# jiaxi98/cnf_ot

Hardware: AMD Instinct MI355X
Metric: MC samples/sec through flow fwd+log|detJ| at dim=2, batch=65536 (higher is better)
Workload: dtype f32; 1 GPU; configs[1]: OT free dim=2, batch=65536, sample_and_log_prob (RQS fwd + log|detJ|), L=2 H=16 M=2 K=5, params N(0,0.20^2) seed 42; ONE STEP = one evaluator-shaped pass of 10000 time-slices x 65536 samples (cnf_ot/utils.py:311-340), each slice its own condition t, one cnf_sample_logprob call per rank; batch=65536, dim=2, parallelism=slice-shard x1 (contiguous blocks of the step's slices; no collective)

## Files before the change

cnf_ot_amd/csrc/cnf_flow.hip:

```cpp
#include "cnf_flow_tile.h"
#include "cnf_host.h"
#include "cnf_pwl_build.h"

#include <math.h>
#include <new>
#include <stdlib.h>
#include <string.h>

namespace cnf {

__global__ void circular_slopes_kernel(const float* __restrict__ params, float* __restrict__ prep, int K, int H,
                                       int D, int L, int M, int64_t per_layer) {
  const int P = 3 * K + 1;
  const int hdr = hdr_floats(K);
  const int l = blockIdx.x / (D - 1), d = 1 + blockIdx.x % (D - 1);
  int64_t o = (int64_t)l * per_layer;
  for (int dd = 1; dd < d; ++dd) o += cond_floats_p(dd, H, M, P, true);
  o += cond_floats_p(d, H, M, P, true) - ((int64_t)H * P + P);
  for (int r = threadIdx.x; r <= H; r += blockDim.x)
    prep[hdr + o + (int64_t)r * P + 3 * K] = params[P + o + (int64_t)r * P + 2 * K];
}

__global__ void prepare_kernel(const float* __restrict__ params, float* __restrict__ prep,
                               int K, int64_t n_params, double lo, double hi, double min_bin,
// ... 213 lines not shown
      const bool odd = l & 1;
      const int first_idx = odd ? D - 1 : 0, idx_step = odd ? -1 : 1;
      const float* cu = U + SPL * lane;
      float* co = O + SPL * lane;
      T o, ld;
      if (wave == 0) {
        table_spline<K, true, FAST, T>(tab, lds_get<T>(cu, first_idx, TS), sc, o, ld);
        lds_put(co, first_idx, TS, o);
        acc += ld;
      }
      for (int d = 1 + wave; d < D; d += NW) {
        const int64_t off = l * a.m.per_layer + (int64_t)H * ((d - 1) + (int64_t)d * (d - 1) / 2) + (d - 1) * cpart;
        T th[P];
        conditioner<H, P, T>(weights + off, d, a.m.M, c, cu, first_idx, idx_step, TS, th);
        const int idx = first_idx + d * idx_step;
        cond_spline<K, true, FAST, T>(th, lds_get<T>(cu, idx, TS), sc, o, ld);
        lds_put(co, idx, TS, o);
        acc += ld;
      }
      __syncthreads();
      float* t = U; U = O; O = t;
    }
    if (a.aux) lds_put(LD + wave * TS + SPL * lane, 0, TS, acc);
    __syncthreads();
    if (a.aux && wave == 0) {
      T tot = splat<T>(0.0f);
      for (int w = 0; w < NW; ++w) tot += lds_get<T>(LD + w * TS + SPL * lane, 0, TS);
      store_aux(a.aux, i, a.B, a.aux_mode == AUX_LOGPROB ? base - tot : tot);
    }
    if (a.out) tile_store_n<float>(a.out, U, D, a.div_magic, TS, tile_start, a.B, NT);
  }
}

struct PwlArgs {
  ModelArgs m;
  const float* in;
  float* out;
  float* aux;
  const float* tables;
  int64_t B, slice_len;
  int32_t n_slices, tiles_per_slice, aux_mode;
  const uint32_t* gate;
  uint32_t gate_epoch;
  int32_t gate_want;
  uint64_t seed;
  int64_t first_sample, slice_stride;
  int32_t in_shared;
};

__global__ void cond_uniform_kernel(const float* __restrict__ c, int64_t B, uint32_t* flag, uint32_t epoch) {
  const uint32_t c0 = __float_as_uint(c[0]);
  bool diff = false;
  for (int64_t i = blockIdx.x * (int64_t)blockDim.x + threadIdx.x; i < B; i += (int64_t)gridDim.x * blockDim.x)
    diff |= __float_as_uint(c[i]) != c0;
  if (__syncthreads_or(diff) && threadIdx.x == 0) *flag = epoch;
}

template <int K, bool TO_BASE, bool FAST, bool PRECISE = false, int LROWS = PWL_LROWS, int LFIX = 0, bool SEEDED = false>
__global__ __launch_bounds__(PWL_MAX_THREADS) void flow_pwl_kernel(const PwlArgs a) {
  const int PWL_THREADS = blockDim.x, PWL_TS = 2 * PWL_THREADS;
  extern __shared__ __attribute__((aligned(16))) float lds_raw[];
  constexpr int HDR = (hdr_floats(K) + 3) & ~3;
  float* tab = lds_raw;
  float* tbl = lds_raw + HDR;
  const int tid = threadIdx.x;
  const int L = LFIX ? LFIX : a.m.L;
  if (gate_closed(a)) return;
  for (int i = tid; i < hdr_floats(K); i += PWL_THREADS) tab[i] = table_of<float>(a.m)[i];
  const SplineConsts sc = sc_scalars(sc_of<float>(a.m));
  [[maybe_unused]] double* e2tab = nullptr;
  [[maybe_unused]] double* tabd = nullptr;
  if constexpr (PRECISE) {
    e2tab = reinterpret_cast<double*>(tbl + L * pwl_ltbl(LROWS));
    tabd = e2tab + EXP2_N;
    for (int i = tid; i < EXP2_N; i += PWL_THREADS) e2tab[i] = a.m.e2tab[i];
    for (int i = tid; i < hdr_floats(K); i += PWL_THREADS) tabd[i] = a.m.tabd[i];
  }

  const int total = a.n_slices * a.tiles_per_slice;
  const int per_block = (total + gridDim.x - 1) / gridDim.x;
  const int t0 = blockIdx.x * per_block;
  const int t1 = t0 + per_block < total ? t0 + per_block : total;
  int cur = -1;
  struct Tile { int slice; int ti; int valid; int64_t g0; int64_t st0; int64_t gin; };
  auto tile_at = [&](int slice, int ti) {
    Tile t;
    t.slice = slice;
    t.ti = ti;
    const int64_t s0 = (int64_t)t.slice * a.slice_len;
    const int64_t len = a.B - s0 < a.slice_len ? a.B - s0 : a.slice_len;
    const int64_t jt = (int64_t)ti * PWL_TS;
    const int64_t left = len - jt;
    t.valid = left >= PWL_TS ? PWL_TS : (left > 0 ? (int)left : 0);
    t.g0 = s0 + jt;
    t.gin = a.in_shared ? jt : t.g0;
    t.st0 = a.first_sample + (int64_t)t.slice * a.slice_stride + jt;
    return t;
  };
  auto tile_of = [&](int tile) { const int sl = tile / a.tiles_per_slice; return tile_at(sl, tile - sl * a.tiles_per_slice); };
  auto tile_next = [&](const Tile& t) {
    return t.ti + 1 < a.tiles_per_slice ? tile_at(t.slice, t.ti + 1) : tile_at(t.slice + 1, 0);
  };
  const uint32_t lane2 = 2u * (uint32_t)tid;
  auto tile_points = [&](const Tile& t) {
    f4 x = {0.f, 0.f, 0.f, 0.f};
    if (SEEDED && !a.in) {
      const uint64_t e0 = (uint64_t)(t.st0 + lane2) * 2u;
      if ((int)lane2 < t.valid) {
        if ((e0 & 3) == 0) {
          float z[4];
          philox_normals4(a.seed, e0 >> 2, z);
#pragma unroll
          for (int q = 0; q < 4; ++q) x[q] = z[q];
        } else {
#pragma unroll
          for (int q = 0; q < 4; ++q) x[q] = normal_at(a.seed, e0 + q);
        }
        if ((int)lane2 + 1 >= t.valid) { x[2] = 0.f; x[3] = 0.f; }
      }
      return x;
    }
    const float* p = a.in + 2 * t.gin;
    if (t.valid == PWL_TS) x = *reinterpret_cast<const f4*>(p + 2u * lane2);
    else if ((int)lane2 + 1 < t.valid) x = *reinterpret_cast<const f4*>(p + 2u * lane2);
    else if ((int)lane2 < t.valid) { x[0] = p[2u * lane2]; x[1] = p[2u * lane2 + 1]; }
    return x;
  };
  [[maybe_unused]] f4 xn = {0.f, 0.f, 0.f, 0.f};
  Tile tn{};
  if (t0 < t1) { tn = tile_of(t0); xn = tile_points(tn); }
  for (int tile = t0; tile < t1; ++tile) {
    const Tile tl = tn;
    const int slice = tl.slice;
    if (slice != cur) {
      __syncthreads();
      pwl_stage<LROWS>(tbl, a.tables + (int64_t)slice * L * PWL_TBL, L, tid, PWL_THREADS);
      cur = slice;
      __syncthreads();
    }
    const bool full = tl.valid == PWL_TS;
    const bool v0 = (int)lane2 < tl.valid, v1 = (int)lane2 + 1 < tl.valid;
    const f4 x = xn;
    if (tile + 1 < t1) { tn = tile_next(tl); xn = tile_points(tn); }
    __builtin_amdgcn_sched_barrier(0);
    v2f u0 = {x[0], x[2]}, u1 = {x[1], x[3]};
    [[maybe_unused]] v2f poison = splat<v2f>(0.0f);
    if constexpr (TO_BASE) poison = (u0 - u0) + (u1 - u1);

    v2f base = splat<v2f>(0.0f);
    if (!TO_BASE && a.aux_mode == AUX_LOGPROB && a.aux) base = (u0 * u0 + u1 * u1) * -0.5f - (float)(2 * HALF_LOG_2PI);
    BaseAcc<v2f> bacc;
    const v2f acc = flow2_tables<K, TO_BASE, FAST, PRECISE, true, LROWS, LFIX, true>(tab, tbl, a.tables + (int64_t)slice * L * PWL_TBL, L, sc,
                                                            u0, u1, &a.m.scd, e2tab, tabd, &bacc);
    if (a.aux) {
      v2f r = acc;
      if constexpr (PRECISE) { if (a.aux_mode == AUX_LOGPROB) r = bacc.log_prob(acc, 2); }
      else if (a.aux_mode == AUX_LOGPROB)
        r = TO_BASE ? (u0 * u0 + u1 * u1) * -0.5f - (float)(2 * HALF_LOG_2PI) + acc : base - acc;
      if constexpr (TO_BASE) r += poison;
      float* q = a.aux + tl.g0;
      if (full || v1) *reinterpret_cast<v2f*>(q + lane2) = r;
      else if (v0) q[lane2] = r.x;
    }
    if (a.out) {
      float* q = a.out + 2 * tl.g0;
      if constexpr (TO_BASE) { u0 += poison; u1 += poison; }
      if (full || v1) *reinterpret_cast<f4*>(q + 2u * lane2) = f4{u0.x, u1.x, u0.y, u1.y};
      else if (v0) { q[2u * lane2] = u0.x; q[2u * lane2 + 1] = u1.x; }
    }
  }
}

struct LossArgs {
  ModelArgs m;
  CnfLossSpec spec;
  const float* pts;
  const float* t;
  double* sums;
  int64_t B;
  int64_t n_slices;
  int64_t pts_slice_stride;
  uint32_t div_magic;
  uint64_t seed;
  int64_t first_sample;
  DensityMix mix;
};

template <class T>
__device__ __forceinline__ void copy_cols(float* dst, const float* src, int D, int TS) {
  for (int d = 0; d < D; ++d) lds_put(dst, d, TS, lds_get<T>(src, d, TS));
}

__device__ __forceinline__ float mask_tail(float v, int64_t i, int64_t B) { return i < B ? v : 0.0f; }
__device__ __forceinline__ float mask_tail(v2f v, int64_t i, int64_t B) {
  return (i < B ? v.x : 0.0f) + (i + 1 < B ? v.y : 0.0f);
}

template <int H, int K, bool FAST, class T>
__global__ __launch_bounds__(TILE, 2) void loss_kernel(const LossArgs a) {
  extern __shared__ __attribute__((aligned(16))) float lds[];
  constexpr int HDR = hdr_floats(K);
  constexpr int SPL = Lanes<T>::N;
  constexpr int TS = TILE * SPL;
  using M = Math<FAST>;
  const int D = a.m.D;
  float* tab = lds;
  float* Nn = lds + HDR;
  float* U = Nn + D * TS;
  float* O = U + D * TS;
  float* V = O + D * TS;
  float* R = V + D * TS;
  for (int i = threadIdx.x; i < HDR; i += TILE) tab[i] = a.m.prep[i];
  const int col = SPL * threadIdx.x;
  const int kind = a.spec.kind;

  const int64_t tiles_per_slice = (a.B + TS - 1) / TS;
  const int64_t n_tiles = tiles_per_slice * a.n_slices;
  SliceSum ssum;
  for (int64_t tile = blockIdx.x; tile < n_tiles; tile += gridDim.x) {
    const int64_t slice = tile / tiles_per_slice;
    const int64_t tile_start = (tile - slice * tiles_per_slice) * TS;
    const int64_t i = tile_start + col;
    __syncthreads();
    if (a.pts)
      tile_load<float>(a.pts + slice * a.pts_slice_stride * D, Nn, D, a.div_magic, TS, tile_start, a.B);
    else
      tile_noise(a.seed, (uint64_t)(a.first_sample + slice * a.pts_slice_stride + tile_start) * (uint64_t)D, Nn, D,
                 a.div_magic, TS, a.B - tile_start);
    const float t = a.t[slice];
    __syncthreads();

    T acc = splat<T>(0.0f);
    const float dt = a.spec.dt;
    const bool kin = kind <= CNF_TERM_FLOW_MATCHING;
    const bool data = kind == CNF_TERM_NEG_LOGPROB || kind == CNF_TERM_DENSITY_L2_DATA;
    const int n_fwd = data ? 0 : (kind == CNF_TERM_KINETIC ? 2 : (kin ? 3 : 1));
    T fldj = splat<T>(0.0f);
    for (int p = 0; p < n_fwd; ++p) {
      const float c = !kin ? t : (p == 0 ? t - 0.5f * dt : (p == 1 ? t + 0.5f * dt : t));
      copy_cols<T>(U + col, Nn + col, D, TS);
      fldj = flow_pass<H, K, false, FAST, T>(a.m, tab, U, O, splat<T>(c));
      if (kin) {
        if (p == 0) copy_cols<T>(V + col, U + col, D, TS);
        else if (p == 1) {
          const float inv_dt = 1.0f / dt;
          for (int d = 0; d < D; ++d)
            lds_put(V + col, d, TS, (lds_get<T>(U + col, d, TS) - lds_get<T>(V + col, d, TS)) * inv_dt);
        } else copy_cols<T>(R + col, U + col, D, TS);
      }
    }
    if (kind == CNF_TERM_KINETIC) {
// ... 448 lines not shown
                  spl == 2 ? CNF_PATH_MLP2 : CNF_PATH_MLP1, gated, a.B);
  });
}

struct SlicePlan { int64_t tps, chunk; float* tables; };

static int slice_plan(CnfModel* m, hipStream_t stream, int64_t slice_len, int64_t n_slices, int64_t tile,
                      int sets_per_slice, SlicePlan* p) {
  const int64_t PWL_MAX_SLICES = 2048;
  p->tps = (slice_len + tile - 1) / tile;
  const int64_t total = n_slices * p->tps;
  if (total > (1 << 30)) return CNF_ERR_UNSUPPORTED;
  if (m->use_pwl == 1 && (total < 2 * (int64_t)m->num_cus || slice_len < 4 * tile)) return CNF_ERR_UNSUPPORTED;
  p->chunk = n_slices < PWL_MAX_SLICES ? n_slices : PWL_MAX_SLICES;
  int64_t sets = 0;
  pwl_workspace(m, stream, &p->tables, &sets);
  if (sets / sets_per_slice < p->chunk) p->chunk = sets / sets_per_slice;
  if (p->chunk < 1) return CNF_ERR_UNSUPPORTED;
  if (m->use_pwl == 1 && p->chunk < n_slices && p->chunk * p->tps < (int64_t)m->num_cus) return CNF_ERR_UNSUPPORTED;
  return CNF_OK;
}

constexpr int64_t PWL_LEAN_MIN_TABLES = 2048;
static void build_tables(CnfModel* m, hipStream_t stream, const float* c, float offset, int64_t ns, float* tables) {
  const int L = m->cfg.num_layers;
  const float* w = m->prep + cnf::hdr_floats(5);
  const bool lean = m->pwl_builder == 0 ? ns * L >= PWL_LEAN_MIN_TABLES : m->pwl_builder != 1;
  m->last_pwl_builder = lean ? 2 : 1;
  const dim3 grid((unsigned)(ns * L));
  if (!lean)
    hipLaunchKernelGGL(cnf::pwl_build_kernel, grid, dim3(512), 0, stream, w, m->per_layer, c, offset, L,
                       m->scd.sp_offset, tables);
  else
    hipLaunchKernelGGL(cnf::pwl_build_lean_kernel<64>, grid, dim3(64), 0, stream, w, m->per_layer, c, offset, L,
                       m->scd.sp_offset, tables);
}

typedef void (*PwlKernel)(const cnf::PwlArgs);

template <bool TO_BASE, bool PRECISE, bool SEEDED>
static PwlKernel flow_pwl_kernel_of(bool full, bool l2) {
  constexpr int ALL = cnf::PWL_NPIECE, WIN = cnf::PWL_LROWS;
  if (l2) return cnf::flow_pwl_kernel<5, TO_BASE, true, PRECISE, ALL, 2, SEEDED>;
  return full ? cnf::flow_pwl_kernel<5, TO_BASE, true, PRECISE, ALL, 0, SEEDED>
              : cnf::flow_pwl_kernel<5, TO_BASE, true, PRECISE, WIN, 0, SEEDED>;
}
static PwlKernel flow_pwl_kernel_of(bool to_base, bool precise, bool seeded, bool full, bool l2) {
  if (precise) return flow_pwl_kernel_of<true, true, false>(full, l2);
  if (to_base) return flow_pwl_kernel_of<true, false, false>(full, l2);
  return seeded ? flow_pwl_kernel_of<false, false, true>(full, l2) : flow_pwl_kernel_of<false, false, false>(full, l2);
}

struct NoiseSrc { uint64_t seed; int64_t first_sample, slice_stride; };

static int run_flow_pwl(CnfModel* m, bool to_base, const float* in, const float* c, int64_t c_block,
                        float* out, float* aux, int aux_mode, int64_t B, hipStream_t stream,
                        bool detect = false, const uint32_t** gate = nullptr, uint32_t* gate_epoch = nullptr,
                        const NoiseSrc* noise = nullptr, const float* built = nullptr, bool in_shared = false) {
  if (!pwl_config_ok(m)) return CNF_ERR_UNSUPPORTED;
  const int L = m->cfg.num_layers;
  const bool precise = to_base && m->precise;
  auto lds_for = [&](int lrows) {
    return (size_t)(((cnf::hdr_floats(5) + 3) & ~3) + L * cnf::pwl_ltbl(lrows)) * sizeof(float) +
           (precise ? precise_lds_bytes(5) : 0);
  };
  const bool full = lds_for(cnf::PWL_NPIECE) <= 160 * 1024;
  size_t lds = lds_for(full ? cnf::PWL_NPIECE : cnf::PWL_LROWS);
  if (lds > 160 * 1024) return CNF_ERR_UNSUPPORTED;
  const int64_t slice_len = c_block < B ? c_block : B;
  const int64_t n_slices = (B + slice_len - 1) / slice_len;
  if (n_slices > 1 && (slice_len & 1)) return CNF_ERR_UNSUPPORTED;
  if ((reinterpret_cast<uintptr_t>(in) & 15) || (reinterpret_cast<uintptr_t>(out) & 15) ||
      (reinterpret_cast<uintptr_t>(aux) & 7))
    return CNF_ERR_UNSUPPORTED;
  const int pwl_threads = cnf::PWL_MAX_THREADS;
  const size_t pwl_min_lds = 82 * 1024;
  SlicePlan plan;
  if (slice_plan(m, stream, slice_len, n_slices, 2 * pwl_threads, 1, &plan) != CNF_OK) return CNF_ERR_UNSUPPORTED;
  const int64_t tps = plan.tps, chunk = plan.chunk;
  float* tables = plan.tables;
  if (built && (chunk < n_slices || built != tables)) return CNF_ERR_UNSUPPORTED;
  if (pwl_min_lds > lds) lds = pwl_min_lds;
  const PwlKernel kern = flow_pwl_kernel_of(to_base, precise, noise != nullptr, full, full && L == 2);
  if (!ensure_lds(kern, lds)) return CNF_ERR_UNSUPPORTED;
  uint32_t* flag = nullptr;
  uint32_t epoch = 0;
  if (detect) {
    int64_t sets = 0;
    pwl_workspace(m, stream, &tables, &sets, &flag, &epoch);
    int64_t g = (B + 4095) / 4096;
    if (g > 4 * (int64_t)m->num_cus) g = 4 * (int64_t)m->num_cus;
    hipLaunchKernelGGL(cnf::cond_uniform_kernel, dim3((unsigned)g), dim3(256), 0, stream, c, B, flag, epoch);
    *gate = flag; *gate_epoch = epoch;
  }
  m->last_path = detect ? CNF_PATH_DETECT : CNF_PATH_TABLES;
  for (int64_t s0 = 0; s0 < n_slices; s0 += chunk) {
    const int64_t ns = n_slices - s0 < chunk ? n_slices - s0 : chunk;
    const int64_t first = s0 * slice_len;
    ProfScope ps(m, stream, true, (B - first) < ns * slice_len ? (B - first) : ns * slice_len, CNF_PATH_TABLES);
    if (!built) build_tables(m, stream, c + s0, 0.0f, ns, tables);
    ps.built();
    cnf::PwlArgs a;
    a.m = model_args(m);
    a.in_shared = in_shared ? 1 : 0;
    a.in = in ? in + (in_shared ? 0 : first * 2) : nullptr; a.out = out ? out + first * 2 : nullptr; a.aux = aux ? aux + first : nullptr;
    a.seed = noise ? noise->seed : 0; a.slice_stride = noise ? noise->slice_stride : 0;
    a.first_sample = noise ? noise->first_sample + s0 * noise->slice_stride : 0;
    a.tables = tables;
    a.B = (B - first) < ns * slice_len ? (B - first) : ns * slice_len;
    a.slice_len = slice_len;
    a.n_slices = (int32_t)ns; a.tiles_per_slice = (int32_t)tps; a.aux_mode = aux_mode;
    a.gate = flag; a.gate_epoch = epoch; a.gate_want = 0;
    const int64_t tiles = ns * tps;
    const int64_t want = (int64_t)m->num_cus;
    const int64_t grid = tiles < want ? tiles : want;
    hipLaunchKernelGGL(kern, dim3((unsigned)grid), dim3(pwl_threads), lds, stream, a);
    ps.done();
  }
  return hipGetLastError() == hipSuccess ? CNF_OK : CNF_ERR_HIP;
}

int cnf_internal_flow_shared(CnfModel* m, hipStream_t stream, const float* in, const float* c, int64_t slice_len,
                             int64_t n_slices, const float* tables, float* out) {
  return run_flow_pwl(m, false, in, c, slice_len, out, nullptr, 0, n_slices * slice_len, stream, false, nullptr, nullptr,
                      nullptr, tables, true);
}

int cnf_internal_build_tables(CnfModel* m, hipStream_t stream, const float* c, int64_t n, float** tables) {
  if (!pwl_config_ok(m) || n < 1) return CNF_ERR_UNSUPPORTED;
  int64_t sets = 0;
  pwl_workspace(m, stream, tables, &sets);
  if (sets < n) return CNF_ERR_UNSUPPORTED;
  build_tables(m, stream, c, 0.0f, n, *tables);
  return hipGetLastError() == hipSuccess ? CNF_OK : CNF_ERR_HIP;
}

extern "C" int cnf_internal_build_tables_into(CnfModel* m, void* stream, const float* c, float c_offset, int64_t n,
                                              float* out) {
  if (!m || !c || !out || n < 1 || n * m->cfg.num_layers > (1 << 30)) return CNF_ERR_INVALID;
  if (!m->params_set) return CNF_ERR_INVALID;
  if (!pwl_network(m->cfg) || (reinterpret_cast<uintptr_t>(out) & 15)) return CNF_ERR_UNSUPPORTED;
  if (wait_for_params(m, (hipStream_t)stream) != CNF_OK) return CNF_ERR_HIP;
  build_tables(m, (hipStream_t)stream, c, c_offset, n, out);
  return hipGetLastError() == hipSuccess ? CNF_OK : CNF_ERR_HIP;
}

template <class R>
static FlowArgsT<R> flow_args(const CnfModel* m, const R* in, const R* c, int64_t c_block, R* out, R* aux, int aux_mode,
                              int64_t B, int64_t tile_samples) {
  FlowArgsT<R> a;
  a.m = model_args(m);
  a.in = in; a.c = c; a.out = out; a.aux = aux;
  a.B = B; a.c_block = c_block; a.aux_mode = aux_mode; a.div_magic = m->div_magic;
  if (c_block >= B) a.c_mode = C_SINGLE;
  else if (c_block == 1) a.c_mode = C_PER_SAMPLE;
  else if (c_block % tile_samples == 0) a.c_mode = C_TILE_UNIFORM;
  else a.c_mode = C_GENERIC;
  a.gate = nullptr; a.gate_epoch = 0; a.gate_want = 0;
  a.fd2 = 0; a.fd_h = 0; a.fd_inv_dx = 0;
  a.seed = 0; a.first_sample = 0; a.slice_stride = 0;
  return a;
}

static int run_flow(CnfModel* m, bool to_base, const float* in, const float* c, int64_t c_block,
                    float* out, float* aux, int aux_mode, int64_t B, void* stream, const NoiseSrc* noise = nullptr) {
  if (!m || (!in && !noise) || (in && noise) || !c || B < 0 || c_block < 1) return CNF_ERR_INVALID;
// ... 314 lines not shown
```

cnf_ot_amd/csrc/cnf_flow_tile.h:

```cpp
#pragma once
#include "cnf_common.h"
#include "cnf_pwl.h"

namespace cnf {

enum CMode { C_SINGLE = 0, C_PER_SAMPLE = 1, C_TILE_UNIFORM = 2, C_GENERIC = 3 };
enum AuxMode { AUX_LOGDET = 0, AUX_LOGPROB = 1 };


template <class R> struct FlowArgsT {
  ModelArgs m;
  const R* in;
  const R* c;
  R* out;
  R* aux;
  int64_t B;
  int64_t c_block;
  int32_t c_mode, aux_mode;
  int32_t div_magic;
  const uint32_t* gate;
  uint32_t gate_epoch;
  int32_t gate_want;
  int32_t fd2;
  R fd_h, fd_inv_dx;
// ... 158 lines not shown
    T o, ld, olo;
    const bool last = step == a.L - 1;
    [[maybe_unused]] R* clo = nullptr;
    if constexpr (PRECISE) {
      clo = LO + SPL * threadIdx.x;
      const T vlo = step == 0 ? splat<T>(0.0f) : lds_get<T>(clo, first_idx, TS);
      table_spline_precise<K, FAST>(tab, tabd, lds_get<T>(cu, first_idx, TS), vlo, sc, o, ld, olo);
      lds_put(clo, first_idx, TS, olo);
      if (last) bacc->add(o, olo);
    } else {
      table_spline<K, INV, FAST, T>(tab, lds_get<T>(cu, first_idx, TS), sc, o, ld);
    }
    lds_put(co, first_idx, TS, o);
    acc += ld;
    uniform_ptr w = weights + l * a.per_layer;
    const float* wq = a.wq + l * a.per_layer_q;
    for (int d = 1; d < D; ++d) {
      const int i = first_idx + d * idx_step;
      T th[P];
      if constexpr (MFMA && !std::is_same<T, double>::value) {
        conditioner_mfma<T>(reinterpret_cast<const f4*>(wq), d, a.M, c, TO_BASE ? co : cu, first_idx, idx_step, TS, th,
                            D >= 3 ? w : nullptr);
        wq += cond_floats_mfma(d, a.M);
        w += cond_floats(d, H, a.M, P);
      } else {
        conditioner<H, P, T, PERIODIC>(w, d, a.M, c, TO_BASE ? co : cu, first_idx, idx_step, TS, th);
        w += cond_floats_p(d, H, a.M, P, PERIODIC);
      }
      if constexpr (PRECISE) {
        const T vlo = step == 0 ? splat<T>(0.0f) : lds_get<T>(clo, i, TS);
        cond_spline_precise<K, FAST, false>(th, lds_get<T>(cu, i, TS), vlo, sc, a.scd, e2tab, o, ld, olo);
        lds_put(clo, i, TS, olo);
        if (last) bacc->add(o, olo);
      } else {
        cond_spline<K, INV, FAST, T>(th, lds_get<T>(cu, i, TS), sc, o, ld);
      }
      lds_put(co, i, TS, o);
      acc += ld;
    }
    R* t = U; U = O; O = t;
  }
  return acc;
}

__device__ __forceinline__ void store_aux(float* aux, int64_t i, int64_t B, float r) {
  if (i < B) aux[i] = r;
}
__device__ __forceinline__ void store_aux(double* aux, int64_t i, int64_t B, double r) {
  if (i < B) aux[i] = r;
}
__device__ __forceinline__ void store_aux(float* aux, int64_t i, int64_t B, v2f r) {
  if (i + 1 < B && ((reinterpret_cast<uintptr_t>(aux + i) & 7) == 0)) *reinterpret_cast<v2f*>(aux + i) = r;
  else { if (i < B) aux[i] = r.x; if (i + 1 < B) aux[i + 1] = r.y; }
}

template <class R>
__device__ __forceinline__ void tile_load_n(const R* __restrict__ g, R* U, int D, uint32_t magic, int TS,
                                            int64_t tile_start, int64_t B, int nthreads) {
  const int64_t base = tile_start * D;
  const int n_el = (int)(B - tile_start < TS ? B - tile_start : TS) * D;
  for (int e = threadIdx.x; e < TS * D; e += nthreads) {
    const int s = magic ? (int)__umulhi((uint32_t)e, magic) : e, d = e - s * D;
    U[d * TS + s] = e < n_el ? g[base + e] : (R)0;
  }
}
template <class R>
__device__ __forceinline__ void tile_store_n(R* __restrict__ g, const R* U, int D, uint32_t magic, int TS,
                                             int64_t tile_start, int64_t B, int nthreads) {
  const int64_t base = tile_start * D;
  const int n_el = (int)(B - tile_start < TS ? B - tile_start : TS) * D;
  for (int e = threadIdx.x; e < n_el; e += nthreads) {
    const int s = magic ? (int)__umulhi((uint32_t)e, magic) : e, d = e - s * D;
    g[base + e] = U[d * TS + s];
  }
}

constexpr int PWL_MAX_THREADS = 1024;

template <int K, bool TO_BASE, bool FAST, bool PRECISE = false, bool SHIFT_FREE_OK = false, int LROWS = PWL_LROWS, int LFIX = 0,
          bool LEAN_OK = false>
__device__ __forceinline__ v2f flow2_tables(const float* tab, const float* tbl, const float* __restrict__ gtbl,
                                            int L, const SplineConsts sc, v2f& u0, v2f& u1,
                                            const PreciseConsts* pc = nullptr, const double* e2tab = nullptr,
                                            const double* tabd = nullptr, BaseAcc<v2f>* bacc = nullptr) {
  constexpr bool INV = !TO_BASE;
  constexpr bool LEAN = LEAN_OK && INV && FAST;
  static_assert(!PRECISE || TO_BASE, "precise path: data -> base");
  v2f acc = splat<v2f>(0.0f);
  [[maybe_unused]] v2f lo0 = splat<v2f>(0.0f), lo1 = lo0;
  if (LFIX) L = LFIX;
#pragma unroll
  for (int step = 0; step < (LFIX ? LFIX : L); ++step) {
    const int l = TO_BASE ? L - 1 - step : step;
    const bool odd = l & 1;
    const v2f uf = odd ? u1 : u0, uo = odd ? u0 : u1;
    v2f of, oo, ld, olo_f, olo_o;
    bool general;
    const float* tl = tbl + l * pwl_ltbl(LROWS);
    const float* gl = gtbl + (int64_t)l * PWL_TBL;
    if constexpr (PRECISE) {
      table_spline_precise<K, FAST>(tab, tabd, uf, odd ? lo1 : lo0, sc, of, ld, olo_f);
      if (step == L - 1) bacc->add(of, olo_f);
      acc += ld;
      v2f th[PWL_P];
      pwl_eval<LROWS>(tl, gl, of, th, general);
      cond_spline_precise<K, FAST, true>(th, uo, odd ? lo0 : lo1, sc, *pc, e2tab, oo, ld, olo_o);
      if (step == L - 1) bacc->add(oo, olo_o);
      lo0 = odd ? olo_o : olo_f;
      lo1 = odd ? olo_f : olo_o;
    } else {
      PwlRows rr;
      v2f qa[K], qb[K];
      if (!TO_BASE) {
        pwl_find<LROWS>(tl, uf, rr, general);
        rr.dua = pwl_logit_pairs<LROWS>(rr.ra, gl, rr.pa, uf.x, qa);
        rr.dub = pwl_logit_pairs<LROWS>(rr.rb, gl, rr.pb, uf.y, qb);
      }
      constexpr bool LOGPROD = LEAN;
      bool tails = true;
      if constexpr (LEAN) tails = __builtin_amdgcn_ballot_w64(maybe_outside(uf, uo, sc.lo, sc.hi)) != 0;
      v2f larg = splat<v2f>(1.0f);
      if constexpr (LOGPROD) {
        table_spline<K, INV, FAST, v2f, true, LEAN>(tab, uf, sc, of, larg, tails);
      } else {
        table_spline<K, INV, FAST, v2f, false, LEAN>(tab, uf, sc, of, ld, tails);
        acc += ld;
      }
      if (TO_BASE) {
        pwl_find<LROWS>(tl, of, rr, general);
        rr.dua = pwl_logit_pairs<LROWS>(rr.ra, gl, rr.pa, of.x, qa);
        rr.dub = pwl_logit_pairs<LROWS>(rr.rb, gl, rr.pb, of.y, qb);
      }
      auto slopes = [&](int ka, int kb, v2f& ta, v2f& tb) {
        ta = pwl_slope_pair<LROWS>(rr.ra, gl, rr.pa, ka, rr.dua);
        tb = pwl_slope_pair<LROWS>(rr.rb, gl, rr.pb, kb, rr.dub);
      };
      if (!SHIFT_FREE_OK || __builtin_amdgcn_ballot_w64(general) != 0)
      {
        cond_spline_rows<K, INV, FAST, false, false, LEAN>(qa, qb, slopes, uo, sc, oo, ld, tails);
        if constexpr (LOGPROD) { const v2f lg = Math<FAST>::log(larg); ld += INV ? -lg : lg; }
      } else {
        cond_spline_rows<K, INV, FAST, true, LOGPROD, LEAN>(qa, qb, slopes, uo, sc, oo, ld, tails);
        if constexpr (LOGPROD) { const v2f lg = Math<FAST>::log(larg * ld); ld = INV ? -lg : lg; }
      }
    }
    acc += ld;
    u0 = odd ? oo : of;
    u1 = odd ? of : oo;
  }
  return acc;
}

}
```

cnf_ot_amd/csrc/cnf_pwl.h:

```cpp
#pragma once

#include "cnf_common.h"

namespace cnf {

constexpr int PWL_H = 16;
constexpr int PWL_P = 16;
constexpr int PWL_NBP = 320;
constexpr int PWL_NG = 2048;
constexpr int PWL_NPIECE = 289;
constexpr float PWL_GMIN = -16.0f;
constexpr float PWL_GSCALE = 64.0f;
constexpr uint32_t PWL_G_INDEX = 0x1ff, PWL_G_MANY = 0x4000, PWL_G_GENERAL = 0x8000;
constexpr int PWL_NREF = 304;
constexpr int PWL_OFF_GRID = PWL_NBP;
constexpr int PWL_OFF_REF = PWL_NBP + PWL_NG / 2;
constexpr int PWL_OFF_PIECE = PWL_NBP + PWL_NG / 2 + PWL_NREF;
static_assert(PWL_OFF_PIECE % 4 == 0, "rows are read with 16-byte LDS loads");
constexpr int PWL_ROW = 36;
constexpr int PWL_TBL = PWL_OFF_PIECE + PWL_NPIECE * PWL_ROW;
constexpr int PWL_LROWS = 112;
constexpr int PWL_LTBL = PWL_OFF_PIECE + PWL_LROWS * PWL_ROW;
constexpr int pwl_ltbl(int lrows) { return PWL_OFF_PIECE + lrows * PWL_ROW; }
constexpr int PWL_N_SLOT = PWL_NBP - 1;
// ... 107 lines not shown
  asm volatile("" : "+v"(q9));
  return (lds_f_ptr)(uintptr_t)((uint32_t)(uintptr_t)(tbl + PWL_OFF_PIECE) + (q9 << 4));
}

template <int LROWS>
__device__ __forceinline__ void pwl_find(const float* tbl, v2f u, PwlRows& r, bool& general) {
  int px, py;
  pwl_piece(tbl, u, px, py, general);
  r.pa = px; r.pb = py;
  r.ra = pwl_lds_row<LROWS>(tbl, px);
  r.rb = pwl_lds_row<LROWS>(tbl, py);
}

template <class FP, class F4P, class V2P>
__device__ __forceinline__ float pwl_logit_pairs_(FP r, F4P r4, V2P r2, float u, v2f (&q)[5]) {
  const f4 s0 = r4[0], s1 = r4[1], t0 = r4[4], t1 = r4[5];
  const v2f s2 = r2[4], t2 = r2[12];
  const float du = u - r[2 * PWL_P];
  const v2f d2 = v2f{du, du};
  q[0] = __builtin_elementwise_fma(__builtin_shufflevector(s0, s0, 0, 1), d2, __builtin_shufflevector(t0, t0, 0, 1));
  q[1] = __builtin_elementwise_fma(__builtin_shufflevector(s0, s0, 2, 3), d2, __builtin_shufflevector(t0, t0, 2, 3));
  q[2] = __builtin_elementwise_fma(__builtin_shufflevector(s1, s1, 0, 1), d2, __builtin_shufflevector(t1, t1, 0, 1));
  q[3] = __builtin_elementwise_fma(__builtin_shufflevector(s1, s1, 2, 3), d2, __builtin_shufflevector(t1, t1, 2, 3));
  q[4] = __builtin_elementwise_fma(s2, d2, t2);
  return du;
}

template <int LROWS>
__device__ __forceinline__ float pwl_logit_pairs(lds_f_ptr row, const float* __restrict__ gtbl, int p, float u,
                                                 v2f (&q)[5]) {
  float du = pwl_logit_pairs_(row, (lds_f4_ptr)row, (lds_v2_ptr)row, u, q);
  if (LROWS < PWL_NPIECE && p >= LROWS) {
    const float* g = gtbl + PWL_OFF_PIECE + p * PWL_ROW;
    du = pwl_logit_pairs_(g, reinterpret_cast<const f4*>(g), reinterpret_cast<const v2f*>(g), u, q);
  }
  return du;
}

template <int LROWS>
__device__ __forceinline__ v2f pwl_slope_pair(lds_f_ptr row, const float* __restrict__ gtbl, int p, int k, float du) {
  const v2f d2 = v2f{du, du};
  const lds_f_ptr r = row + k;
  v2f t = __builtin_elementwise_fma(v2f{r[10], r[11]}, d2, v2f{r[PWL_P + 10], r[PWL_P + 11]});
  if (LROWS < PWL_NPIECE && p >= LROWS) {
    const float* g = gtbl + PWL_OFF_PIECE + p * PWL_ROW + k;
    t = __builtin_elementwise_fma(v2f{g[10], g[11]}, d2, v2f{g[PWL_P + 10], g[PWL_P + 11]});
  }
  return t;
}

template <int LROWS, int NT>
__device__ __forceinline__ float pwl_row_dot(lds_f_ptr row, const float* __restrict__ gtbl, int p, int k,
                                             const float (&t)[NT], float s0, float s1) {
  static_assert(NT == 10, "K = 5");
  auto dot = [&](f4 a, f4 b, v2f c, float k0, float k1) {
    float r = k0 * s0;
    r = fmaf(k1, s1, r);
#pragma unroll
    for (int e = 0; e < 4; ++e) { r = fmaf(a[e], t[e], r); r = fmaf(b[e], t[4 + e], r); }
    r = fmaf(c.x, t[8], r);
    return fmaf(c.y, t[9], r) * 0.693147182464599609375f;
  };
  const lds_f_ptr rk = row + k;
  float r = dot(((lds_f4_ptr)row)[0], ((lds_f4_ptr)row)[1], ((lds_v2_ptr)row)[4], rk[10], rk[11]);
  if (LROWS < PWL_NPIECE && p >= LROWS) {
    const float* g = gtbl + PWL_OFF_PIECE + p * PWL_ROW;
    r = dot(reinterpret_cast<const f4*>(g)[0], reinterpret_cast<const f4*>(g)[1], reinterpret_cast<const v2f*>(g)[4], g[10 + k], g[11 + k]);
  }
  return r;
}

template <int LROWS = PWL_LROWS>
__device__ __forceinline__ void pwl_stage(float* tbl, const float* __restrict__ g0, int L, int tid, int nthreads) {
  for (int l = 0; l < L; ++l) {
    const float* g = g0 + (int64_t)l * PWL_TBL;
    const int n = __float_as_int(g[PWL_N_SLOT]);
    const int rows = n + 1 < LROWS ? n + 1 : LROWS;
    const f4* src = reinterpret_cast<const f4*>(g);
    f4* dst = reinterpret_cast<f4*>(tbl + l * pwl_ltbl(LROWS));
    for (int i = tid; i < (PWL_OFF_PIECE + rows * PWL_ROW) / 4; i += nthreads) dst[i] = src[i];
  }
}

}
```

Before: 88.54 billion samples/s.

## Double-buffer per-slice PWL tables in LDS with async global-to-LDS prefetch

For the L=2 inverse non-precise path, LDS is split into two compact table images. While the current slice's tiles are processed, the next slice's tables are prefetched asynchronously with global_load_lds, so only a waitcnt and a barrier are needed at each slice switch. This is meant to hide the synchronous table staging and the double __syncthreads at each slice boundary, given 10000 slices per step. It adds a per-slice LDS stride parameter and a compact image layout that is only used when row counts fit, raises the LDS request to about 160KB, and falls back to the old staging otherwise.

```diff
diff --git a/cnf_ot_amd/csrc/cnf_flow.hip b/cnf_ot_amd/csrc/cnf_flow.hip
--- a/cnf_ot_amd/csrc/cnf_flow.hip
+++ b/cnf_ot_amd/csrc/cnf_flow.hip
@@ -319,6 +319,12 @@
   const int t0 = blockIdx.x * per_block;
   const int t1 = t0 + per_block < total ? t0 + per_block : total;
   int cur = -1;
+  constexpr bool DB = LFIX == 2 && LROWS >= PWL_NPIECE && !TO_BASE && !PRECISE;
+  [[maybe_unused]] const int last_slice = t0 < t1 ? (t1 - 1) / a.tiles_per_slice : -1;
+  [[maybe_unused]] int img = 0;
+  int lstr = pwl_ltbl(LROWS);
+  [[maybe_unused]] int pf = 0;
+  [[maybe_unused]] const int wave = __builtin_amdgcn_readfirstlane(tid >> 6);
   struct Tile { int slice; int ti; int valid; int64_t g0; int64_t st0; int64_t gin; };
   auto tile_at = [&](int slice, int ti) {
     Tile t;
@@ -370,10 +376,34 @@
     const Tile tl = tn;
     const int slice = tl.slice;
     if (slice != cur) {
-      __syncthreads();
-      pwl_stage<LROWS>(tbl, a.tables + (int64_t)slice * L * PWL_TBL, L, tid, PWL_THREADS);
-      cur = slice;
-      __syncthreads();
+      if constexpr (DB) {
+        const float* gs = a.tables + (int64_t)slice * 2 * PWL_TBL;
+        if (pf == 2) {
+          asm volatile("s_waitcnt vmcnt(0)" ::: "memory");
+          __syncthreads();
+          img = PWL_IMG - img;
+        } else {
+          __syncthreads();
+          const int n0 = __builtin_amdgcn_readfirstlane(__float_as_int(gs[PWL_N_SLOT]));
+          const int n1 = __builtin_amdgcn_readfirstlane(__float_as_int(gs[PWL_TBL + PWL_N_SLOT]));
+          img = 0;
+          if (pwl_image_fits(n0, n1)) {
+            pwl_copy_image(tbl, gs, pwl_image(n0, n1), tid, PWL_THREADS);
+            lstr = PWL_SUB;
+          } else {
+            pwl_stage<LROWS>(tbl, gs, 2, tid, PWL_THREADS);
+            lstr = pwl_ltbl(LROWS);
+          }
+          __syncthreads();
+        }
+        cur = slice;
+        pf = slice < last_slice && lstr == PWL_SUB ? 1 : 0;
+      } else {
+        __syncthreads();
+        pwl_stage<LROWS>(tbl, a.tables + (int64_t)slice * L * PWL_TBL, L, tid, PWL_THREADS);
+        cur = slice;
+        __syncthreads();
+      }
     }
     const bool full = tl.valid == PWL_TS;
     const bool v0 = (int)lane2 < tl.valid, v1 = (int)lane2 + 1 < tl.valid;
@@ -387,8 +417,8 @@
     v2f base = splat<v2f>(0.0f);
     if (!TO_BASE && a.aux_mode == AUX_LOGPROB && a.aux) base = (u0 * u0 + u1 * u1) * -0.5f - (float)(2 * HALF_LOG_2PI);
     BaseAcc<v2f> bacc;
-    const v2f acc = flow2_tables<K, TO_BASE, FAST, PRECISE, true, LROWS, LFIX, true>(tab, tbl, a.tables + (int64_t)slice * L * PWL_TBL, L, sc,
-                                                            u0, u1, &a.m.scd, e2tab, tabd, &bacc);
+    const v2f acc = flow2_tables<K, TO_BASE, FAST, PRECISE, true, LROWS, LFIX, true>(tab, DB ? tbl + img : tbl, a.tables + (int64_t)slice * L * PWL_TBL, L, sc,
+                                                            u0, u1, &a.m.scd, e2tab, tabd, &bacc, lstr);
     if (a.aux) {
       v2f r = acc;
       if constexpr (PRECISE) { if (a.aux_mode == AUX_LOGPROB) r = bacc.log_prob(acc, 2); }
@@ -404,6 +434,18 @@
       if constexpr (TO_BASE) { u0 += poison; u1 += poison; }
       if (full || v1) *reinterpret_cast<f4*>(q + 2u * lane2) = f4{u0.x, u1.x, u0.y, u1.y};
       else if (v0) { q[2u * lane2] = u0.x; q[2u * lane2 + 1] = u1.x; }
+    }
+    if constexpr (DB) {
+      if (pf == 1) {
+        const uniform_ptr gn = as_uniform(a.tables + (int64_t)(slice + 1) * 2 * PWL_TBL);
+        const int n0 = __float_as_int(gn[PWL_N_SLOT]), n1 = __float_as_int(gn[PWL_TBL + PWL_N_SLOT]);
+        pf = 0;
+        if (pwl_image_fits(n0, n1)) {
+          pwl_copy_image_async(tbl + (PWL_IMG - img), a.tables + (int64_t)(slice + 1) * 2 * PWL_TBL, pwl_image(n0, n1), wave,
+                               tid & 63, PWL_THREADS >> 6);
+          pf = 2;
+        }
+      }
     }
   }
 }
@@ -1018,6 +1060,8 @@
   if (built && (chunk < n_slices || built != tables)) return CNF_ERR_UNSUPPORTED;
   if (pwl_min_lds > lds) lds = pwl_min_lds;
   const PwlKernel kern = flow_pwl_kernel_of(to_base, precise, noise != nullptr, full, full && L == 2);
+  if (full && L == 2 && !to_base)
+    lds = (size_t)(((cnf::hdr_floats(5) + 3) & ~3) + 2 * cnf::PWL_IMG) * sizeof(float);
   if (!ensure_lds(kern, lds)) return CNF_ERR_UNSUPPORTED;
   uint32_t* flag = nullptr;
   uint32_t epoch = 0;
diff --git a/cnf_ot_amd/csrc/cnf_flow_tile.h b/cnf_ot_amd/csrc/cnf_flow_tile.h
--- a/cnf_ot_amd/csrc/cnf_flow_tile.h
+++ b/cnf_ot_amd/csrc/cnf_flow_tile.h
@@ -264,7 +264,8 @@
 __device__ __forceinline__ v2f flow2_tables(const float* tab, const float* tbl, const float* __restrict__ gtbl,
                                             int L, const SplineConsts sc, v2f& u0, v2f& u1,
                                             const PreciseConsts* pc = nullptr, const double* e2tab = nullptr,
-                                            const double* tabd = nullptr, BaseAcc<v2f>* bacc = nullptr) {
+                                            const double* tabd = nullptr, BaseAcc<v2f>* bacc = nullptr,
+                                            const int lstride = pwl_ltbl(LROWS)) {
   constexpr bool INV = !TO_BASE;
   constexpr bool LEAN = LEAN_OK && INV && FAST;
   static_assert(!PRECISE || TO_BASE, "precise path: data -> base");
@@ -278,7 +279,7 @@
     const v2f uf = odd ? u1 : u0, uo = odd ? u0 : u1;
     v2f of, oo, ld, olo_f, olo_o;
     bool general;
-    const float* tl = tbl + l * pwl_ltbl(LROWS);
+    const float* tl = tbl + l * lstride;
     const float* gl = gtbl + (int64_t)l * PWL_TBL;
     if constexpr (PRECISE) {
       table_spline_precise<K, FAST>(tab, tabd, uf, odd ? lo1 : lo0, sc, of, ld, olo_f);
diff --git a/cnf_ot_amd/csrc/cnf_pwl.h b/cnf_ot_amd/csrc/cnf_pwl.h
--- a/cnf_ot_amd/csrc/cnf_pwl.h
+++ b/cnf_ot_amd/csrc/cnf_pwl.h
@@ -213,4 +213,54 @@
   }
 }
 
-}
+constexpr int PWL_LDS_FLOATS = 160 * 1024 / 4;
+constexpr int PWL_WAVE_ITEMS = 64;
+constexpr int pwl_sub(int hdr) { return (PWL_LDS_FLOATS - hdr) / 4 / (4 * PWL_WAVE_ITEMS) * (4 * PWL_WAVE_ITEMS); }
+constexpr int PWL_SUB = pwl_sub((hdr_floats(5) + 3) & ~3);
+constexpr int PWL_SUB_ROWS = (PWL_SUB - PWL_OFF_PIECE) / PWL_ROW;
+constexpr int PWL_IMG = 2 * PWL_SUB;
+static_assert(PWL_SUB % 4 == 0 && PWL_TBL % 4 == 0, "images are copied in 16-byte items");
+static_assert(2 * PWL_IMG >= 2 * pwl_ltbl(PWL_NPIECE), "the two images hold one slice with every row");
+
+struct PwlImage { int c0, total; };
+__device__ __forceinline__ bool pwl_image_fits(int n0, int n1) {
+  return n0 >= 0 && n0 < PWL_SUB_ROWS && n1 >= 0 && n1 < PWL_SUB_ROWS;
+}
+__device__ __forceinline__ PwlImage pwl_image(int n0, int n1) {
+  PwlImage im;
+  auto items = [](int n) { return ((PWL_OFF_PIECE + (n + 1) * PWL_ROW) / 4 + PWL_WAVE_ITEMS - 1) & ~(PWL_WAVE_ITEMS - 1); };
+  im.c0 = items(n0);
+  im.total = im.c0 + items(n1);
+  return im;
+}
+__device__ __forceinline__ const f4* pwl_item_src(const float* __restrict__ g, PwlImage im, int i) {
+  return reinterpret_cast<const f4*>(g) + (i < im.c0 ? i : i - im.c0 + PWL_TBL / 4);
+}
+__device__ __forceinline__ f4* pwl_item_dst(float* img, PwlImage im, int i) {
+  return reinterpret_cast<f4*>(img) + (i < im.c0 ? i : i - im.c0 + PWL_SUB / 4);
+}
+__device__ __forceinline__ void pwl_copy_image(float* img, const float* __restrict__ g, PwlImage im, int first,
+                                               int nthreads) {
+  for (int i = first; i < im.total; i += 2 * nthreads) {
+    const int j = i + nthreads;
+    const bool two = j < im.total;
+    const f4 a = *pwl_item_src(g, im, i), b = *pwl_item_src(g, im, two ? j : i);
+    *pwl_item_dst(img, im, i) = a;
+    if (two) *pwl_item_dst(img, im, j) = b;
+  }
+}
+
+__device__ __forceinline__ void pwl_copy_image_async(float* img, const float* __restrict__ g, PwlImage im, int wave,
+                                                     int lane, int nwaves) {
+  typedef const __attribute__((address_space(1))) void* gptr;
+  typedef __attribute__((address_space(3))) void* lptr;
+  for (int ib = wave * PWL_WAVE_ITEMS; ib < im.total; ib += nwaves * PWL_WAVE_ITEMS) {
+    const bool l1 = ib >= im.c0;
+    const int j = l1 ? ib - im.c0 : ib;
+    const float* src = g + (l1 ? PWL_TBL : 0) + 4 * (j + lane);
+    float* dst = img + (l1 ? PWL_SUB : 0) + 4 * j;
+    __builtin_amdgcn_global_load_lds((gptr)src, (lptr)(uintptr_t)(uint32_t)(uintptr_t)dst, 16, 0, 0);
+  }
+}
+
+}
```

After: 88.76 billion samples/s, median of 6. No clear change (+0.2%).
